# Gavinli-lgf/belief-planning

Hardware: AMD Instinct MI355X
Metric: branch-MPC solves/sec (whole node), highway N=20 M=3 branches, batch 4096 egos (higher is better)
Workload: dtype f64; 1 GPU; highway BranchMPC_CVaR closed loop, N=20, NB=1, m=3 (T=64, U=61), 4096 egos per GPU; batch_per_gpu=4096, global_batch=4096, world_size=1, parallelism=ego-sharded dp1, loop=per step: k_env + solve launches

## Files before the change

belief-planning_amd/csrc/bmpc_core.h:

```cpp
#pragma once

#include <stddef.h>
#include <stdint.h>

#include "bmpc.h"

#if defined(__HIPCC__)
#include <hip/hip_runtime.h>
#define BMPC_HD __host__ __device__ __forceinline__
#if defined(BMPC_INLINE_ALL)
#define BMPC_FN __host__ __device__ __forceinline__
#else
#define BMPC_FN __host__ __device__ __attribute__((noinline))
#endif
#else
#define BMPC_HD inline
#define BMPC_FN inline
#endif

#include <math.h>

namespace bmpc {

#if defined(__HIP_DEVICE_COMPILE__)
#if defined(BMPC_FLAT_SLAB)
#define BMPC_AS_GLOBAL
#else
#define BMPC_AS_GLOBAL __attribute__((address_space(1)))
#endif
#define BMPC_AS_LDS __attribute__((address_space(3)))
#define BMPC_AS_CONST __attribute__((address_space(4)))
#else
#define BMPC_AS_GLOBAL
#define BMPC_AS_LDS
#define BMPC_AS_CONST
#endif
typedef BMPC_AS_GLOBAL double gdouble;
typedef BMPC_AS_LDS double ldouble;
typedef const BMPC_AS_GLOBAL int32_t gint;

template <class T>
BMPC_HD T* uniform_ptr(T* p) {
#if defined(__HIP_DEVICE_COMPILE__)
  const uint64_t v = reinterpret_cast<uint64_t>(p);
  const uint32_t lo = __builtin_amdgcn_readfirstlane(static_cast<uint32_t>(v));
  const uint32_t hi = __builtin_amdgcn_readfirstlane(static_cast<uint32_t>(v >> 32));
  return reinterpret_cast<T*>((static_cast<uint64_t>(hi) << 32) | lo);
#else
  return p;
#endif
}

#define BMPC_TOPO_FIELDS(F)                                                                  \
  F(br_depth) F(br_len) F(br_ndx) F(br_ndu) F(br_child0) F(x_u) F(x_srcu) F(x_srcx) F(x_cone) \
  F(x_conepos) F(x_branch) F(succ_off) F(succ) F(lvl_off) F(lvl_nodes) F(u_x) F(u_cone)       \
  F(cone_b) F(cone_i) F(cone_c) F(cone_q) F(cone_off)
#define BMPC_TOPO_COUNT_(n) +1
enum { BMPC_TOPO_N = 0 BMPC_TOPO_FIELDS(BMPC_TOPO_COUNT_) };
#define BMPC_TOPO_MEMBER_(n) IP n;
template <class IP>
struct TopoT {
  BMPC_TOPO_FIELDS(BMPC_TOPO_MEMBER_)
};
typedef const BMPC_AS_LDS int32_t lint;
typedef TopoT<gint*> Topo;
typedef TopoT<lint*> TopoL;

enum { XF_S = 0, XF_BX = BMPC_MAX_N * BMPC_MAX_N, XF_SON = XF_BX + BMPC_MAX_FX, XF_BXSET = XF_SON + 1,
       XF_FX = XF_BXSET + 1, XF_FXSET = XF_FX + BMPC_MAX_FX * BMPC_MAX_N, XF_ROWS = XF_FXSET + 1,
       XF_BROWS = XF_ROWS + BMPC_MAX_FX * BMPC_MAX_N, XF_ROWSET = XF_BROWS + BMPC_MAX_FX,
       XF_COUNT = XF_ROWSET + 1 };

enum { ECO_FX = 0, ECO_W1 = BMPC_MAX_FX * BMPC_MAX_N, ECO_QQ = ECO_W1 + BMPC_MAX_N * BMPC_MAX_N,
       ECO_BX = ECO_QQ + BMPC_MAX_N * BMPC_MAX_N, ECO_COUNT = ECO_BX + BMPC_MAX_FX };

struct Plan {
  bmpc_plan_desc desc;
  int n, d, N, NB, m, nFx, nFu, Nc;
  int Ncol, zNB;
  int T, U, nbranch, bdim, ncones, nlevels;
  int oX, oU, oRho, oSig, oMup, oMum, oS, oJ, nv;
  int neq;
  int rFx, rFu, rRisk, rPos, nlp, nrows;
  int ng;
  int nsm;
  int lds_M, lds_piv, lds_rhs, lds_rhs2, lds_red, nlds;
  int lds_w, lds_wu, lds_fx, lds_fu, nconst;
  int nlds_lean;
  int lds_scr, nscr;
  int cgrp;
  int maxq;
  double W1[BMPC_MAX_N * BMPC_MAX_N];
  double Wu[BMPC_MAX_D * BMPC_MAX_D];
  double QQ[BMPC_MAX_N * BMPC_MAX_N];
  double RR[BMPC_MAX_D * BMPC_MAX_D];
  Topo t;
  int toff[BMPC_TOPO_N];
  int ntab;
  const double* lref;
  int nlref;
};

template <class X>
// ... 343 lines not shown
```

belief-planning_amd/csrc/bmpc_ipm.h:

```cpp
#pragma once

#include <type_traits>

#include "bmpc_tree.h"
#include "bmpc_wave.h"

#ifndef BMPC_EQUIL
#define BMPC_EQUIL 1
#endif
#ifndef BMPC_EQUIL_ITERS
#define BMPC_EQUIL_ITERS 3
#endif
#ifndef BMPC_TS_POST_RB_MIN
#define BMPC_TS_POST_RB_MIN 8
#endif
#ifndef BMPC_TS_POST_RB
#define BMPC_TS_POST_RB 4
#endif
#ifndef BMPC_PAIR_REFINE
#define BMPC_PAIR_REFINE 1
#endif
#ifndef BMPC_BLK_WAVE_SUBST
#define BMPC_BLK_WAVE_SUBST 1
#endif
// ... 37 lines not shown
#define BMPC_REFSCORE 1e-3
#endif
#ifndef BMPC_REFSCORE2
#define BMPC_REFSCORE2 1e-6
#endif
#ifndef BMPC_NITREF2
#define BMPC_NITREF2 2
#endif
#ifndef BMPC_REFTOL
#define BMPC_REFTOL 1e-14
#endif
#ifndef BMPC_REF_STALL
#define BMPC_REF_STALL 0
#endif

#ifndef BMPC_FN_APPLY_G
#define BMPC_FN_APPLY_G BMPC_FN
#endif
#ifndef BMPC_FN_APPLY_GT
#define BMPC_FN_APPLY_GT BMPC_FN
#endif
#ifndef BMPC_FN_SCALING
#define BMPC_FN_SCALING BMPC_FN
#endif
#ifndef BMPC_FN_MAX_STEP
#define BMPC_FN_MAX_STEP BMPC_FN
#endif
#ifndef BMPC_FN_TREE_SOLVE
#define BMPC_FN_TREE_SOLVE BMPC_FN
#endif
#ifndef BMPC_FN_FUSED
#define BMPC_FN_FUSED BMPC_FN
#endif

namespace bmpc {

enum {
  EXIT_OPTIMAL = 0, EXIT_PINF = 1, EXIT_DINF = 2, EXIT_INACC = 10,
  EXIT_MAXIT = -1, EXIT_NUMERICS = -2,
  EXIT_GUARD = -9
};

struct Ctx {
  CPlan* P;
  CLayout* L;
  gdouble* ws;
  BMPC_HD gdouble* at(size_t off) const { return ws + off; }
  BMPC_HD Ctx uniform() const { return Ctx{uniform_ptr(P), uniform_ptr(L), uniform_ptr(ws)}; }
};

template <int NX>
BMPC_HD void ctx_qx(const Ctx& C, double (&qx)[NX]) {
  const gdouble* xref = C.at(C.L->xref);
  double xr[NX];
#pragma unroll
  for (int r = 0; r < NX; ++r) xr[r] = xref[r];
#pragma unroll
  for (int c = 0; c < NX; ++c) {
    double v = 0.0;
#pragma unroll
    for (int r = 0; r < NX; ++r) v += xr[r] * C.P->desc.Q[r * NX + c];
    qx[c] = v;
  }
}

#define BMPC_CONE_ROUNDS(ex, P, G)                                \
  const auto G##_t = topo_view((P), ex);                         \
  const ConeGroups G = cone_groups(ex, (P).cgrp, (P).ncones);     \
  for (int rnd_ = 0; rnd_ < G.rounds; ++rnd_)
#define BMPC_CONE_K(P, G, k, off, q)                              \
  const int k = rnd_ * G.ngrp + G.g < (P).ncones ? rnd_ * G.ngrp + G.g : -1; \
  const int off = k >= 0 ? G##_t.cone_off[k] : 0;                 \
  const int q = k >= 0 ? G##_t.cone_q[k] : 0

template <class X>
struct MultiWave : std::integral_constant<bool, (BatchDiv<X>::v > 1)> {};

template <class X, class PB>
BMPC_HD double ebeta(const PB* boost, int nc, int k) {
  if constexpr (MultiWave<X>::value) return boost[nc + k];
  return exp(-boost[k]);
}

template <int NBR0 = 4, class X>
BMPC_HD void block_dots(const X ex, const gdouble* A, size_t astr, int na, const gdouble* B, size_t bstr, int nb,
                        int lo1, int hi1, int lo2, int hi2, double (&acc)[4][4]) {
  constexpr int NBR = MultiWave<X>::value ? NBR0 : 4;
#pragma unroll
  for (int a = 0; a < 4; ++a)
#pragma unroll
    for (int b = 0; b < 4; ++b) acc[a][b] = 0.0;
  const int n1 = hi1 - lo1, ntot = n1 + (hi2 - lo2);
  auto idx = [&](int t) { return t < n1 ? lo1 + t : lo2 + (t - n1); };
#pragma unroll 2
  for (int t = ex.lane; t < ntot; t += ex.nlanes) {
    const int i = idx(t);
    double av[4], bv[4];
#pragma unroll
    for (int a = 0; a < 4; ++a) av[a] = a < na ? A[a * astr + i] : 0.0;
#pragma unroll
    for (int b = 0; b < 4; ++b) bv[b] = b < nb ? B[b * bstr + i] : 0.0;
#pragma unroll
    for (int a = 0; a < 4; ++a)
#pragma unroll
      for (int b = 0; b < (NBR < 4 ? NBR : 4); ++b) acc[a][b] += av[a] * bv[b];
  }
  if constexpr (NBR >= 4) {
    ex.template sum_n<16>(&acc[0][0]);
  } else {
    double v[4 * NBR];
#pragma unroll
    for (int a = 0; a < 4; ++a)
#pragma unroll
      for (int b = 0; b < NBR; ++b) v[a * NBR + b] = acc[a][b];
    ex.template sum_n<4 * NBR>(v);
#pragma unroll
    for (int a = 0; a < 4; ++a)
#pragma unroll
      for (int b = 0; b < NBR; ++b) acc[a][b] = v[a * NBR + b];
  }
}

template <class T>
BMPC_HD int cone_supp_len(CPlan& P, const T& t, int k) {
  return t.cone_c[k] >= 0 ? P.N * (P.n + P.d + P.Nc) : P.d + P.Nc;
}
template <class T>
BMPC_HD int cone_supp_idx(CPlan& P, const T& t, int k, int e) {
  const int c = t.cone_c[k];
  if (c < 0) return e < P.d ? P.oU + e : P.oS + (e - P.d);
  const int xn = P.N * P.n, un = P.N * P.d;
  if (e < xn) return P.oX + t.br_ndx[c] * P.n + e;
  if (e < xn + un) return P.oU + t.br_ndu[c] * P.d + (e - xn);
  return P.oS + t.br_ndx[c] * P.Nc + (e - xn - un);
}
BMPC_HD bool coup_supp_dots(CPlan& P) { return P.ncones > 4; }

template <class X, class T>
BMPC_HD void cone_supp_dots(const X& ex, CPlan& P, const T& t, const gdouble* gk, int k, const gdouble* v0,
                            size_t vstr, int j0, int nvec, double (&acc)[16]) {
#pragma unroll
  for (int j = 0; j < 16; ++j) acc[j] = 0.0;
  const int tot = cone_supp_len(P, t, k);
  for (int e = ex.lane; e < tot; e += ex.nlanes) {
    const int i = cone_supp_idx(P, t, k, e);
    const double g = gk[i];
    double v[16];
#pragma unroll
    for (int j = 0; j < 16; ++j) v[j] = v0[(size_t)(j0 + j < nvec ? j0 + j : j0) * vstr + i];
#pragma unroll
    for (int j = 0; j < 16; ++j) acc[j] += (j0 + j < nvec ? g : 0.0) * v[j];
  }
  ex.template sum_n<16>(acc);
}

template <class X, class T>
BMPC_HD void cone_supp_gdx(const X& ex, CPlan& P, const T& t, const gdouble* g0, size_t gstr, const gdouble* dx, int k0,
                           double (&acc)[16]) {
#pragma unroll
  for (int j = 0; j < 16; ++j) acc[j] = 0.0;
  const int nc = P.ncones;
  const int kn = nc - k0 < 16 ? nc - k0 : 16;
  const int full = P.N * (P.n + P.d + P.Nc);
  int tot = 0;
  for (int j = 0; j < kn; ++j) tot += cone_supp_len(P, t, k0 + j);
  constexpr int UN = 8;
  for (int b = ex.lane; b < tot; b += UN * ex.nlanes) {
    double gv[UN], xv[UN];
    int kk[UN];
#pragma unroll
    for (int u = 0; u < UN; ++u) {
      const int f = b + u * ex.nlanes < tot ? b + u * ex.nlanes : b;
      const int j = f / full < kn ? f / full : kn - 1;
      const int e = f - j * full;
      const int i = cone_supp_idx(P, t, k0 + j, e);
      kk[u] = b + u * ex.nlanes < tot ? j : -1;
      gv[u] = g0[(size_t)(k0 + j) * gstr + i];
      xv[u] = dx[i];
    }
#pragma unroll
    for (int u = 0; u < UN; ++u)
#pragma unroll
      for (int j = 0; j < 16; ++j) acc[j] += (kk[u] == j ? gv[u] : 0.0) * xv[u];
  }
  ex.template sum_n<16>(acc);
}

template <class X, class T>
BMPC_HD void cone_supp_gdx2(const X& ex, CPlan& P, const T& t, const gdouble* g0, size_t gstr, const gdouble* dx1,
                            const gdouble* dx2, int k0, double (&acc1)[16], double (&acc2)[16]) {
#pragma unroll
  for (int j = 0; j < 16; ++j) acc1[j] = 0.0, acc2[j] = 0.0;
  const int nc = P.ncones;
  const int kn = nc - k0 < 16 ? nc - k0 : 16;
  const int full = P.N * (P.n + P.d + P.Nc);
  int tot = 0;
  for (int j = 0; j < kn; ++j) tot += cone_supp_len(P, t, k0 + j);
  constexpr int UN = 4;
  for (int b = ex.lane; b < tot; b += UN * ex.nlanes) {
    double gv[UN], xv1[UN], xv2[UN];
    int kk[UN];
#pragma unroll
    for (int u = 0; u < UN; ++u) {
// ... 1505 lines not shown
            Pn[q][j] = i == j ? pij : i < j ? 0.5 * (pij + pji) : 0.5 * (pji + pij);
          }
        }
#pragma unroll
        for (int q = 0; q < RX; ++q) {
          const int i = gl * RX + q;
          if (i < NX) {
#pragma unroll
            for (int j = 0; j < NX; ++j) ws[L.P + k * NX * NX + i * NX + j] = Pn[q][j];
#pragma unroll
            for (int m = 0; m < NU; ++m) ws[L.Kg + u * NU * NX + m * NX + i] = kc[q][m];
          }
        }
        if (gl == 0) mat_store(Qi, ws + L.Luu + u * NU * NU);
        BMPC_TOC_WAIT(C.ws, L, PROF_RIC_B, t_rb);
      }
    }
    ex.sync();
  }
  BMPC_TOC(C.ws, L, 23, t_ric);
  return ex.max(bad) == 0.0;
}

template <class X, int NX, int NU, int RX, int W>
BMPC_HD void bw_node(const X& ex, int gl, const double (&qx)[RX], const double (&Acol)[RX][NX],
                     const double (&Brow)[RX][NU], const double (&Kcol)[RX][NU], const double (&Lu)[NU][NU],
                     const double (&ru)[NU], double (&g)[RX], double (&l)[RX], double (&kfv)[NU]) {
#pragma unroll
  for (int q = 0; q < RX; ++q)
    if (gl * RX + q >= NX) g[q] = 0.0;
  double gfull[NX];
  task_gather<NX, RX, W>(ex, g, gfull);
  double qu[NU];
#pragma unroll
  for (int m = 0; m < NU; ++m) {
    double v = 0.0;
#pragma unroll
    for (int q = 0; q < RX; ++q) v += Brow[q][m] * g[q];
    qu[m] = -ru[m] + ex.tsum(v);
  }
#pragma unroll
  for (int m = 0; m < NU; ++m) {
    double v = 0.0;
#pragma unroll
    for (int c = 0; c < NU; ++c) v -= Lu[m][c] * qu[c];
    kfv[m] = v;
  }
#pragma unroll
  for (int q = 0; q < RX; ++q) {
    double v = qx[q];
#pragma unroll
    for (int j = 0; j < NX; ++j) v += Acol[q][j] * gfull[j];
#pragma unroll
    for (int m = 0; m < NU; ++m) v += Kcol[q][m] * qu[m];
    l[q] = v;
  }
}

template <class X, int NX, int NU, bool RB = false>
BMPC_FN_TREE_SOLVE void tree_solve(const X ex, const Ctx Cin, int nr, const gdouble* r0, size_t rs, const gdouble* e0,
                        size_t es, gdouble* o0, size_t os, gdouble* n0, size_t ns, int ncw = 0) {
  const Ctx C = Cin.uniform();
  r0 = uniform_ptr(r0);
  e0 = uniform_ptr(e0);
  o0 = uniform_ptr(o0);
  n0 = uniform_ptr(n0);
  constexpr int W = X::kTaskLanes;
  constexpr int RX = (NX + W - 1) / W;
  constexpr int NCM = BMPC_MAX_FX + 1;
  (void)NCM;
  CPlan& P = *C.P;
  CLayout& L = *C.L;
  BMPC_PROF(C.ws, L, PROF_TREESOLVE);
  BMPC_COUNT(C.ws, L, PROF_NTREE);
  const auto t = topo_view(P, ex);
  const int Nc = P.Nc;
  gdouble* ws = C.ws;
  gdouble* lv_ = ws + L.lvec;
  gdouble* kf_ = ws + L.kff;
  const size_t lstr = (size_t)P.T * NX, kstr = (size_t)P.U * NU;
  const gdouble* dh = ws + L.dh;
  const gdouble* sdv = ws + L.sd;
  const int gl = ex.lane % W, grp = ex.lane / W, ngrp = ex.nlanes / W;
  auto needed = [&](int b, int ri) {
    if (ri >= ncw) return true;
    int c = t.cone_c[ri];
    if (c < 0) return b == 0;
    while (c > b) c = (c - 1) / P.m;
    return c == b;
  };
  auto qx0 = [&](const gdouble* rr, int k, int i) {
    double rS[NCM], s0[NCM], s1[NCM];
#pragma unroll
    for (int c = 0; c < NCM; ++c) {
      const int kc = k * Nc + (c < Nc ? c : 0);
      rS[c] = rr[P.oS + kc];
      s0[c] = sdv[kc * 2];
      s1[c] = sdv[kc * 2 + 1];
    }
    const double on = t.x_u[k] >= 0 ? 1.0 : 0.0;
    double v = -rr[P.oX + k * NX + i] + dh[k * NX + i] * (on * s1[0] * rS[0] / s0[0]);
#pragma unroll
    for (int c = 1; c < NCM; ++c)
      if (c < Nc) v -= fxv(P, ex, c - 1, i) * (on * s1[c] * rS[c] / s0[c]);
    return v;
  };
  const bool pre = ex.uniform(P.nscr >= P.T * Nc);
  gdouble* q0_ = ws + L.qx0;
  if (pre) {
    BMPC_TIC(t_pre);
    ldouble* av = ex.lds + P.lds_scr;
    for (int ri = 0; ri < nr; ++ri) {
      const gdouble* rr = r0 + ri * rs;
      gdouble* q0 = q0_ + ri * lstr;
      int s0 = 0, l0 = P.T, s1 = 0, l1 = 0, s2 = 0, l2 = 0, s3 = 0, l3 = 0;
      if (ri < ncw) {
        int c = t.cone_c[ri] < 0 ? 0 : t.cone_c[ri];
        int st[4] = {0, 0, 0, 0}, ln[4] = {0, 0, 0, 0};
        bool deeper = true;
#pragma unroll
        for (int q = 0; q < 4; ++q) {
          if (deeper) {
            st[q] = t.br_ndx[c];
            ln[q] = t.br_len[c] + (t.br_child0[c] < 0 ? 1 : 0);
            if (c == 0) deeper = false;
            else c = (c - 1) / P.m;
          }
        }
        if (!deeper) s0 = st[0], l0 = ln[0], s1 = st[1], l1 = ln[1], s2 = st[2], l2 = ln[2], s3 = st[3], l3 = ln[3];
      }
      const int nn = l0 + l1 + l2 + l3;
      auto node = [&](int f) {
        const int f1 = f - l0, f2 = f1 - l1, f3 = f2 - l2;
        return f < l0 ? s0 + f : f1 < l1 ? s1 + f1 : f2 < l2 ? s2 + f2 : s3 + f3;
      };
      lane_batch<BMPC_TS_UN_AV>(ex, 0, nn * Nc, [&](int f) {
        const int k = node(f / Nc), it = k * Nc + f % Nc;
        const double on = t.x_u[k] >= 0 ? 1.0 : 0.0;
        return on * sdv[it * 2 + 1] * rr[P.oS + it] / sdv[it * 2];
      }, [&](int f, double v) { av[node(f / Nc) * Nc + f % Nc] = v; });
      ex.sync();
      lane_batch<BMPC_TS_UN>(ex, 0, nn * NX, [&](int f) {
        const int k = node(f / NX), j = f % NX, it = k * NX + j;
        double v = -rr[P.oX + it] + dh[it] * av[k * Nc];
        for (int c = 1; c < Nc; ++c) v -= fxv(P, ex, c - 1, j) * av[k * Nc + c];
        return v;
      }, [&](int f, double v) { q0[node(f / NX) * NX + f % NX] = v; });
      ex.sync();
    }
    BMPC_TOC(C.ws, L, PROF_X1, t_pre);
  }

  BMPC_TIC(t_bw);
  for (int dep = P.NB; dep >= 0; --dep) {
    const int b0 = branch_start(P, dep), nbd = branch_count(P, dep);
    const int nfull = nbd * (nr - ncw);
    int ncol = 0;
    for (int ri = 0; ri < ncw; ++ri) {
      const int c = t.cone_c[ri];
      ncol += (c < 0 ? 0 : t.br_depth[c]) >= dep ? 1 : 0;
    }
    const int ntask = nfull + ncol;
    const int rounds = (ntask + ngrp - 1) / ngrp;
    const bool leaf = dep == P.NB;
    for (int rd = 0; rd < rounds; ++rd) {
      const int task = rd * ngrp + grp;
      if (task >= ntask) continue;
      int b, ri;
      if (task < nfull) {
        b = b0 + task / (nr - ncw);
        ri = ncw + task % (nr - ncw);
      } else {
        int want = task - nfull;
        ri = 0;
        for (int r2 = 0; r2 < ncw; ++r2) {
          const int c = t.cone_c[r2];
          if ((c < 0 ? 0 : t.br_depth[c]) >= dep) {
            if (want == 0) {
              ri = r2;
              break;
            }
            --want;
          }
        }
        int c = t.cone_c[ri];
        if (c < 0) c = 0;
        while (t.br_depth[c] > dep) c = (c - 1) / P.m;
        b = c;
      }
      const gdouble* rr = r0 + ri * rs;
      const gdouble* ee = e0 + ri * es;
      const gdouble* q0 = q0_ + ri * lstr;
      gdouble* lvec = lv_ + ri * lstr;
      gdouble* kf = kf_ + ri * kstr;
      const int ndx = t.br_ndx[b], ndu = t.br_ndu[b], len = t.br_len[b];
      const int c0 = t.br_child0[b];
      double l[RX];
      if (leaf) {
        const int tn = ndx + len;
#pragma unroll
        for (int q = 0; q < RX; ++q) {
          const int i = gl * RX + q;
          l[q] = i < NX ? (pre ? q0[tn * NX + i] : qx0(rr, tn, i)) : 0.0;
          if (i < NX) lvec[tn * NX + i] = l[q];
        }
      }
      for (int jn = len - 1; jn >= 0; --jn) {
        const int k = ndx + jn, u = ndu + jn;
        double qx[RX], Acol[RX][NX], Brow[RX][NU], Kcol[RX][NU], Lu[NU][NU], ru[NU];
#pragma unroll
        for (int q = 0; q < RX; ++q) {
          const int i = gl * RX + q < NX ? gl * RX + q : NX - 1;
          qx[q] = pre ? q0[k * NX + i] : qx0(rr, k, i);
#pragma unroll
          for (int j = 0; j < NX; ++j) Acol[q][j] = ws[L.Ad + u * NX * NX + j * NX + i];
#pragma unroll
          for (int m = 0; m < NU; ++m) Brow[q][m] = ws[L.Bd + u * NX * NU + i * NU + m];
#pragma unroll
          for (int m = 0; m < NU; ++m) Kcol[q][m] = ws[L.Kg + u * NU * NX + m * NX + i];
        }
        mat_load(Lu, ws + L.Luu + u * NU * NU);
#pragma unroll
        for (int m = 0; m < NU; ++m) ru[m] = rr[P.oU + u * NU + m];
        double g[RX];
        if (jn < len - 1 || leaf) {
          double ec[NX];
#pragma unroll
          for (int j = 0; j < NX; ++j) ec[j] = ee[(k + 1) * NX + j];
#pragma unroll
          for (int q = 0; q < RX; ++q) {
            const int i = gl * RX + q < NX ? gl * RX + q : NX - 1;
            double v = l[q];
#pragma unroll
            for (int j = 0; j < NX; ++j) v += ws[L.P + (k + 1) * NX * NX + i * NX + j] * ec[j];
            g[q] = v;
          }
        } else {
#pragma unroll
          for (int q = 0; q < RX; ++q) g[q] = 0.0;
          for (int ci = 0; ci < P.m; ++ci) {
            if (!needed(c0 + ci, ri)) continue;
            const int c = t.br_ndx[c0 + ci];
            double ec[NX];
#pragma unroll
            for (int j = 0; j < NX; ++j) ec[j] = ee[c * NX + j];
#pragma unroll
            for (int q = 0; q < RX; ++q) {
              const int i = gl * RX + q < NX ? gl * RX + q : NX - 1;
              double v = lvec[c * NX + i];
#pragma unroll
              for (int j = 0; j < NX; ++j) v += ws[L.P + c * NX * NX + i * NX + j] * ec[j];
              g[q] += v;
            }
          }
        }
        double kfv[NU];
        bw_node<X, NX, NU, RX, W>(ex, gl, qx, Acol, Brow, Kcol, Lu, ru, g, l, kfv);
#pragma unroll
        for (int q = 0; q < RX; ++q) {
          const int i = gl * RX + q;
          if (i < NX) lvec[k * NX + i] = l[q];
        }
        if (gl == 0)
#pragma unroll
          for (int m = 0; m < NU; ++m) kf[u * NU + m] = kfv[m];
      }
    }
    ex.sync();
  }
  BMPC_TOC(C.ws, L, PROF_X2, t_bw);
  BMPC_TIC(t_fw);
  for (int it = ex.lane; it < nr * NX; it += ex.nlanes) {
    const int ri = it / NX, j = it % NX;
    o0[ri * os + P.oX + j] = e0[ri * es + j];
  }
  ex.sync();
  for (int dep = 0; dep <= P.NB; ++dep) {
    const int b0 = branch_start(P, dep), nbd = branch_count(P, dep);
    const int ntask = nbd * nr;
    const int rounds = (ntask + ngrp - 1) / ngrp;
    const bool leaf = dep == P.NB;
    for (int rd = 0; rd < rounds; ++rd) {
      const int task = rd * ngrp + grp;
      if (task >= ntask) continue;
      const int b = b0 + task / nr, ri = task % nr;
      gdouble* o = o0 + ri * os;
      const gdouble* ee = e0 + ri * es;
      const gdouble* kf = kf_ + ri * kstr;
      const bool kfon = needed(b, ri);
      const int ndx = t.br_ndx[b], ndu = t.br_ndu[b], len = t.br_len[b];
      const int c0 = t.br_child0[b];
      double xk[NX];
#pragma unroll
      for (int j = 0; j < NX; ++j) xk[j] = o[P.oX + ndx * NX + j];
      for (int jn = 0; jn < len; ++jn) {
        const int k = ndx + jn, u = ndu + jn;
        double Arow[RX][NX], Brow[RX][NU], Kcol[RX][NU], kfu[NU], en[RX];
        const int kn = (jn < len - 1 || leaf) ? k + 1 : t.br_ndx[c0 >= 0 ? c0 : 0];
#pragma unroll
        for (int q = 0; q < RX; ++q) {
          const int i = gl * RX + q < NX ? gl * RX + q : NX - 1;
#pragma unroll
          for (int j = 0; j < NX; ++j) Arow[q][j] = ws[L.Ad + u * NX * NX + i * NX + j];
#pragma unroll
          for (int m = 0; m < NU; ++m) Brow[q][m] = ws[L.Bd + u * NX * NU + i * NU + m];
#pragma unroll
          for (int m = 0; m < NU; ++m) Kcol[q][m] = ws[L.Kg + u * NU * NX + m * NX + i];
          en[q] = ee[kn * NX + i];
        }
#pragma unroll
        for (int m = 0; m < NU; ++m) kfu[m] = kfon ? kf[u * NU + m] : 0.0;
        double uk[NU];
#pragma unroll
        for (int m = 0; m < NU; ++m) {
          double v = 0.0;
#pragma unroll
          for (int q = 0; q < RX; ++q) v += gl * RX + q < NX ? Kcol[q][m] * xk[gl * RX + q < NX ? gl * RX + q : 0] : 0.0;
          uk[m] = kfu[m] + ex.tsum(v);
        }
        if (gl == 0)
#pragma unroll
          for (int m = 0; m < NU; ++m) o[P.oU + u * NU + m] = uk[m];
        double xn[RX];
#pragma unroll
        for (int q = 0; q < RX; ++q) {
          double v = 0.0;
#pragma unroll
          for (int j = 0; j < NX; ++j) v += Arow[q][j] * xk[j];
#pragma unroll
          for (int m = 0; m < NU; ++m) v += Brow[q][m] * uk[m];
          xn[q] = v;
        }
        if (jn < len - 1 || leaf) {
#pragma unroll
          for (int q = 0; q < RX; ++q) {
            const int i = gl * RX + q;
            xn[q] += en[q];
            if (i < NX) o[P.oX + (k + 1) * NX + i] = xn[q];
          }
          task_gather<NX, RX, W>(ex, xn, xk);
        } else {
          for (int ci = 0; ci < P.m; ++ci) {
            const int c = t.br_ndx[c0 + ci];
#pragma unroll
            for (int q = 0; q < RX; ++q) {
              const int i = gl * RX + q;
              if (i < NX) o[P.oX + c * NX + i] = xn[q] + ee[c * NX + i];
            }
          }
        }
      }
    }
    ex.sync();
  }
  BMPC_TOC(C.ws, L, PROF_X3, t_fw);
  BMPC_TIC(t_post);
  if constexpr (RB) {
    constexpr int NB4 = BMPC_TS_POST_RB;
    struct VR { double v[NB4]; };
    for (int rb = 0; rb < nr; rb += NB4) {
      const int rn = nr - rb < NB4 ? nr - rb : NB4;
      if (n0) {
        lane_batch<BMPC_TS_UN>(ex, 0, P.T * NX, [&](int it) {
          const int k = it / NX, i = it % NX;
          double pr[NX];
#pragma unroll
          for (int j = 0; j < NX; ++j) pr[j] = ws[L.P + k * NX * NX + i * NX + j];
          VR out;
#pragma unroll
          for (int a = 0; a < NB4; ++a) {
// ... 314 lines not shown
      const int i = i1 - u;
      if (i >= 0) {
        if (j == i) b[i] = b[i] / mc[u];
        wave_sync();
        const double bi = b[i];
        if (row && j < i) b[j] -= mc[u] * bi;
        wave_sync();
      }
    }
  }
}

template <class X, class PM, class PP, class PB>
BMPC_HD void small_lu_solve(const X ex, const PM* M, const PP* piv, PB* b, int n) {
#if BMPC_SUBST_REG
  if constexpr (MultiWave<X>::value) {
    if (n <= 64) {
      PB* const bs[1] = {b};
      if (ex.lane < 64) small_lu_solve_wave<1>(ex.lane, M, piv, bs, n);
      ex.sync();
      return;
    }
  }
#endif
  if (ex.lane == 0)
    for (int k = 0; k < n; ++k) {
      const int p = (int)piv[k];
      if (p != k) {
        const double tmp = b[k];
        b[k] = b[p];
        b[p] = tmp;
      }
    }
  ex.sync();
  if constexpr (RowLanes<X>::value) {
#if BMPC_BLK_WAVE_SUBST
    if constexpr (X::nlanes > 64) {
      if (n <= 64) {
        if (ex.lane < 64) small_lu_solve_rows_wave(ex.lane, M, b, n);
        ex.sync();
        return;
      }
    }
#endif
    if (n <= X::nlanes) {
      small_lu_solve_rows(ex, M, b, n);
      return;
    }
  }
  for (int i = 0; i < n; ++i) {
    const double bi = b[i];
    for (int j = i + 1 + ex.lane; j < n; j += ex.nlanes) b[j] -= M[j * n + i] * bi;
    ex.sync();
  }
  for (int i = n - 1; i >= 0; --i) {
    const double bi = b[i] / M[i * n + i];
    for (int j = ex.lane; j < i; j += ex.nlanes) b[j] -= M[j * n + i] * bi;
    ex.sync();
    if (ex.lane == 0) b[i] = bi;
    ex.sync();
  }
}

template <class X>
BMPC_HD auto coup_mem(const X& ex, gdouble* ws, CLayout& L, CPlan& P, int off) {
  if constexpr (X::kCoupLds) return ex.lds + off;
  else return ws + L.coup + (off - P.lds_M);
}
template <class X>
BMPC_HD auto coup_vec(const X& ex, int off) { return ex.lds + off; }


BMPC_HD int gvar(CPlan& P, int i) { return i == P.ng - 1 ? P.oJ : P.oRho + i; }

template <class X, int NX, int NU>
BMPC_FN bool kkt_coupling(const X ex, const Ctx Cin, int extra) {
  const Ctx C = Cin.uniform();
  CPlan& P = *C.P;
  CLayout& L = *C.L;
  BMPC_PROF(C.ws, L, PROF_COUPLING);
  gdouble* ws = C.ws;
  const int nc = P.ncones;
  BMPC_TIC(t_cts);
  if (ex.uniform(nc + extra >= BMPC_TS_POST_RB_MIN))
    tree_solve<X, NX, NU, true>(ex, C, nc + extra, ws + L.gk, P.nv, ws + L.zeros, P.neq, ws + L.colk, P.nv,
                                ws + L.colnu, P.neq, nc);
  else
    tree_solve<X, NX, NU>(ex, C, nc + extra, ws + L.gk, P.nv, ws + L.zeros, P.neq, ws + L.colk, P.nv, ws + L.colnu,
                          P.neq, nc);
  BMPC_TOC(C.ws, L, PROF_CTS, t_cts);
  BMPC_TIC(t_cdot);
  const int ng = P.ng, nb = P.bdim, ns = P.nsm;
  auto* M = coup_mem(ex, ws, L, P, P.lds_M);
  const gdouble* eta = ws + L.eta;
  const gdouble* dl = ws + L.dl;
  const gdouble* p = ws + L.p;
  const int ntree = P.oRho;
  for (int i = ex.lane; i < ns * ns; i += ex.nlanes) M[i] = 0.0;
  ex.sync();
  if (coup_supp_dots(P) && BMPC_BLK_PAIR_DOTS && MultiWave<X>::value) {
    const auto t = topo_view(P, ex);
    for (int pr = ex.lane; pr < nc * nc; pr += ex.nlanes) {
      const int k = pr / nc, j = pr - (pr / nc) * nc;
      const gdouble* g = ws + L.gk + (size_t)k * P.nv;
      const gdouble* v = ws + L.colk + (size_t)j * P.nv;
      const int tot = cone_supp_len(P, t, k);
      double acc = 0.0;
      for (int e0 = 0; e0 < tot; e0 += 8) {
        double gv[8], vv[8];
#pragma unroll
        for (int u = 0; u < 8; ++u) {
          const int i = cone_supp_idx(P, t, k, e0 + u < tot ? e0 + u : e0);
          gv[u] = g[i];
          vv[u] = v[i];
        }
#pragma unroll
        for (int u = 0; u < 8; ++u)
          if (e0 + u < tot) acc += gv[u] * vv[u];
      }
      const double ck = 2.0 / (eta[k] * eta[k]);
      M[(ng + nb + k) * ns + ng + nb + j] = ck * acc + (k == j ? 1.0 : 0.0);
    }
  } else if (coup_supp_dots(P)) {
    const auto t = topo_view(P, ex);
    for (int k = 0; k < nc; ++k)
      for (int j0 = 0; j0 < nc; j0 += 16) {
        double acc[16];
        cone_supp_dots(ex, P, t, ws + L.gk + (size_t)k * P.nv, k, ws + L.colk, P.nv, j0, nc, acc);
        if (ex.lane == 0) {
          const double ck = 2.0 / (eta[k] * eta[k]);
          for (int j = j0; j < nc && j < j0 + 16; ++j)
            M[(ng + nb + k) * ns + ng + nb + j] = ck * acc[j - j0] + (k == j ? 1.0 : 0.0);
        }
      }
  } else {
    for (int k0 = 0; k0 < nc; k0 += 4)
      for (int j0 = 0; j0 < nc; j0 += 4) {
        const int na = nc - k0 < 4 ? nc - k0 : 4, nbk = nc - j0 < 4 ? nc - j0 : 4;
        double acc[4][4];
        block_dots(ex, ws + L.gk + (size_t)k0 * P.nv, P.nv, na, ws + L.colk + (size_t)j0 * P.nv, P.nv, nbk,
                   0, ntree, P.oS, P.oJ, acc);
        if (ex.lane == 0)
          for (int a = 0; a < na; ++a) {
            const int k = k0 + a;
            const double ck = 2.0 / (eta[k] * eta[k]);
            for (int b = 0; b < nbk; ++b) {
              const int j = j0 + b;
              M[(ng + nb + k) * ns + ng + nb + j] = ck * acc[a][b] + (k == j ? 1.0 : 0.0);
            }
          }
      }
  }
  for (int b = ex.lane; b < nb; b += ex.nlanes) {
    const double w = dl[P.rRisk + b];
    M[b * ns + b] = 1.0 / (w * w);
  }
  for (int j = ex.lane; j < 2 * nb * P.m; j += ex.nlanes) {
    const double w = dl[P.rRisk + nb + j];
    const int gi = 2 * nb + j;
    M[gi * ns + gi] = 1.0 / (w * w);
  }
  for (int b = ex.lane; b < nb; b += ex.nlanes) {
    const int row = ng + b;
    M[row * ns + b] = 1.0;
    M[b * ns + row] = 1.0;
    M[row * ns + nb + b] = 1.0;
    M[(nb + b) * ns + row] = 1.0;
    for (int i = 0; i < P.m; ++i) {
      const int gi = 2 * nb + nb * P.m + b * P.m + i;
      const double a = -p[b * P.m + i] / P.desc.ralpha;
      M[row * ns + gi] = a;
      M[gi * ns + row] = a;
    }
  }
  for (int it = ex.lane; it < nc * ng; it += ex.nlanes) {
    const int k = it / ng, i = it % ng;
    const double gv = ws[L.gk + (size_t)k * P.nv + gvar(P, i)];
    const double ck = 2.0 / (eta[k] * eta[k]);
    M[i * ns + ng + nb + k] = gv;
    M[(ng + nb + k) * ns + i] = -ck * gv;
  }
  ex.sync();
  BMPC_TOC(C.ws, L, PROF_CDOT, t_cdot);
  BMPC_TIC(t_lu);
  bool ok;
  if constexpr (BMPC_WAVE_LU && RowLanes<X>::value && (MultiWave<X>::value || !X::kCoupLds)) {
    if (ns <= 64 && (MultiWave<X>::value || ns >= BMPC_WAVE_LU_MIN1)) {
      double bad = 0.0;
      if (ex.lane < 64) bad = small_lu_wave(ex.lane, M, coup_vec(ex, P.lds_piv), ns) ? 0.0 : 1.0;
      ok = ex.max(bad) == 0.0;
    } else {
      ok = small_lu(ex, M, coup_vec(ex, P.lds_piv), ns);
    }
  } else {
    ok = small_lu(ex, M, coup_vec(ex, P.lds_piv), ns);
  }
  BMPC_TOC(C.ws, L, PROF_LU, t_lu);
  return ok;
}

template <class X, int NX, int NU, bool R3ZERO>
BMPC_HD void kkt_back(const X ex, const Ctx& C, const gdouble* tz, const gdouble* r2, const gdouble* r3h,
                      gdouble* dx, gdouble* dy, gdouble* dzh, bool fin);

template <class X, int NX, int NU, bool R3ZERO = false>
BMPC_HD void kkt_solve_once(const X ex, const Ctx Cin, const gdouble* r1, const gdouble* r2,
                            const gdouble* r3h, gdouble* dx, gdouble* dy, gdouble* dzh, bool tr_ready, bool fin) {
  const Ctx C = Cin.uniform();
  CPlan& P = *C.P;
  CLayout& L = *C.L;
  gdouble* ws = C.ws;
  gdouble* tr = ws + L.k_r0;
  gdouble* tz = ws + L.k_nv0;
  if constexpr (R3ZERO) {
    tz = const_cast<gdouble*>(r1);
  } else {
    if (!tr_ready) apply_W(ex, C, 1, r3h, tr);
    apply_GT<X, NX, NU>(ex, C, tr, tz, r1);
  }
  tree_solve<X, NX, NU>(ex, C, 1, tz, 0, r2, 0, dx, 0, dy, 0);
  kkt_back<X, NX, NU, R3ZERO>(ex, C, tz, r2, r3h, dx, dy, dzh, fin);
}

template <class X, int NX, int NU, bool R3ZERO>
BMPC_HD void kkt_back(const X ex, const Ctx& C, const gdouble* tz, const gdouble* r2, const gdouble* r3h,
                      gdouble* dx, gdouble* dy, gdouble* dzh, bool fin) {
  CPlan& P = *C.P;
  CLayout& L = *C.L;
  BMPC_PROF(C.ws, L, PROF_BACK);
  gdouble* ws = C.ws;
  gdouble* tr = ws + L.k_r0;
  const int ng = P.ng, nb = P.bdim, nc = P.ncones, ns = P.nsm;
  auto* b = coup_vec(ex, P.lds_rhs);
  const gdouble* eta = ws + L.eta;
  if (coup_supp_dots(P)) {
    const auto t = topo_view(P, ex);
    for (int k0 = 0; k0 < nc; k0 += 16) {
      double acc[16];
      cone_supp_gdx(ex, P, t, ws + L.gk, P.nv, dx, k0, acc);
      if (ex.lane == 0)
        for (int a = 0; a < 16 && k0 + a < nc; ++a) b[ng + nb + k0 + a] = 2.0 / (eta[k0 + a] * eta[k0 + a]) * acc[a];
    }
  } else {
    for (int k0 = 0; k0 < nc; k0 += 4) {
      const int na = nc - k0 < 4 ? nc - k0 : 4;
      double acc[4][4];
      block_dots<1>(ex, ws + L.gk + (size_t)k0 * P.nv, P.nv, na, dx, 0, 1, 0, P.oRho, P.oS, P.oJ, acc);
      if (ex.lane == 0)
        for (int a = 0; a < na; ++a) b[ng + nb + k0 + a] = 2.0 / (eta[k0 + a] * eta[k0 + a]) * acc[a][0];
    }
  }
  for (int i = ex.lane; i < ng + nb; i += ex.nlanes) b[i] = i < ng ? tz[gvar(P, i)] : r2[P.T * NX + i - ng];
  ex.sync();
  BMPC_TIC(t_lus);
  small_lu_solve(ex, coup_mem(ex, ws, L, P, P.lds_M), coup_vec(ex, P.lds_piv), b, ns);
  BMPC_TOC(C.ws, L, PROF_LUS, t_lus);
  const auto* bc = b + ng + nb;
  const gdouble* colk = ws + L.colk;
  const gdouble* colnu = ws + L.colnu;
  const int n1 = P.oRho, n2 = n1 + (P.oJ - P.oS), n3 = n2 + P.T * NX;
  auto row = [&](int t, int& i, bool& isx) {
    isx = t < n2;
    i = t < n1 ? t : t < n2 ? P.oS + (t - n1) : t - n2;
  };
  lane_batch(ex, 0, n3, [&](int t) {
    int i;
    bool isx;
    row(t, i, isx);
    const gdouble* col = isx ? colk : colnu;
    const size_t cs = isx ? (size_t)P.nv : (size_t)P.neq;
    const gdouble* src = isx ? dx : dy;
    double v = src[i];
    for (int k0 = 0; k0 < nc; k0 += 4) {
      double c4[4], b4[4];
#pragma unroll
      for (int a = 0; a < 4; ++a) {
        c4[a] = col[(size_t)(k0 + a < nc ? k0 + a : nc - 1) * cs + i];
        b4[a] = k0 + a < nc ? bc[k0 + a] : 0.0;
      }
#pragma unroll
      for (int a = 0; a < 4; ++a) v -= b4[a] * c4[a];
    }
    return v;
  }, [&](int t, double v) {
    int i;
    bool isx;
    row(t, i, isx);
    if (isx) dx[i] = v;
    else dy[i] = v;
  });
  for (int i = ex.lane; i < ng + nb; i += ex.nlanes) {
    if (i < ng) dx[gvar(P, i)] = b[i];
    else dy[P.T * NX + i - ng] = b[i];
  }
  ex.sync();
  if constexpr (R3ZERO) apply_G<X, NX, NU, 3>(ex, C, dx, dzh, r3h, tr);
  else if (fin) apply_G<X, NX, NU, 2>(ex, C, dx, dzh, r3h, tr);
  else apply_G<X, NX, NU, 1>(ex, C, dx, dzh, r3h, tr);
}

template <class X, int NX, int NU, bool R3ZERO = false>
BMPC_HD void kkt_back_pair(const X ex, const Ctx& C, const gdouble* tz1, const gdouble* r21, const gdouble* r3h1,
                           gdouble* dx1, gdouble* dy1, gdouble* dzh1, const gdouble* tz2, const gdouble* r22,
                           const gdouble* r3h2, gdouble* dx2, gdouble* dy2, gdouble* dzh2, bool fin) {
  CPlan& P = *C.P;
  CLayout& L = *C.L;
  BMPC_PROF(C.ws, L, PROF_BACK);
  gdouble* ws = C.ws;
  gdouble* tr = ws + L.k_r0;
  const int ng = P.ng, nb = P.bdim, nc = P.ncones, ns = P.nsm;
  auto* b1 = coup_vec(ex, P.lds_rhs);
  auto* b2 = coup_vec(ex, P.lds_rhs2);
  const gdouble* eta = ws + L.eta;
  if (coup_supp_dots(P)) {
    const auto t = topo_view(P, ex);
    for (int k0 = 0; k0 < nc; k0 += 16) {
      double acc1[16], acc2[16];
      cone_supp_gdx2(ex, P, t, ws + L.gk, P.nv, dx1, dx2, k0, acc1, acc2);
      if (ex.lane == 0)
        for (int a = 0; a < 16 && k0 + a < nc; ++a) {
          b1[ng + nb + k0 + a] = 2.0 / (eta[k0 + a] * eta[k0 + a]) * acc1[a];
          b2[ng + nb + k0 + a] = 2.0 / (eta[k0 + a] * eta[k0 + a]) * acc2[a];
        }
    }
  } else {
    for (int k0 = 0; k0 < nc; k0 += 4) {
      const int na = nc - k0 < 4 ? nc - k0 : 4;
      double acc[4][4];
      block_dots<2>(ex, ws + L.gk + (size_t)k0 * P.nv, P.nv, na, dx1, (size_t)(dx2 - dx1), 2, 0, P.oRho, P.oS, P.oJ,
                 acc);
      if (ex.lane == 0)
        for (int a = 0; a < na; ++a) {
          b1[ng + nb + k0 + a] = 2.0 / (eta[k0 + a] * eta[k0 + a]) * acc[a][0];
          b2[ng + nb + k0 + a] = 2.0 / (eta[k0 + a] * eta[k0 + a]) * acc[a][1];
        }
    }
  }
  for (int i = ex.lane; i < ng + nb; i += ex.nlanes) {
    b1[i] = i < ng ? tz1[gvar(P, i)] : r21[P.T * NX + i - ng];
    b2[i] = i < ng ? tz2[gvar(P, i)] : r22[P.T * NX + i - ng];
  }
  ex.sync();
  BMPC_TIC(t_lus);
  bool both = false;
#if BMPC_SUBST_REG
  if constexpr (MultiWave<X>::value) {
    if (ns <= 64) {
      decltype(b1) const bs[2] = {b1, b2};
      if (ex.lane < 64) small_lu_solve_wave<2>(ex.lane, coup_mem(ex, ws, L, P, P.lds_M), coup_vec(ex, P.lds_piv), bs, ns);
      ex.sync();
      both = true;
    }
  }
#endif
  if (!both) {
    small_lu_solve(ex, coup_mem(ex, ws, L, P, P.lds_M), coup_vec(ex, P.lds_piv), b1, ns);
    small_lu_solve(ex, coup_mem(ex, ws, L, P, P.lds_M), coup_vec(ex, P.lds_piv), b2, ns);
  }
  BMPC_TOC(C.ws, L, PROF_LUS, t_lus);
  const auto* bc1 = b1 + ng + nb;
  const auto* bc2 = b2 + ng + nb;
  const gdouble* colk = ws + L.colk;
  const gdouble* colnu = ws + L.colnu;
  const int n1 = P.oRho, n2 = n1 + (P.oJ - P.oS), n3 = n2 + P.T * NX;
  auto row = [&](int t, int& i, bool& isx) {
    isx = t < n2;
    i = t < n1 ? t : t < n2 ? P.oS + (t - n1) : t - n2;
  };
  struct V2 { double a, b; };
  lane_batch<4>(ex, 0, n3, [&](int t) {
    int i;
    bool isx;
    row(t, i, isx);
    const gdouble* col = isx ? colk : colnu;
    const size_t cs = isx ? (size_t)P.nv : (size_t)P.neq;
    const gdouble* s1 = isx ? dx1 : dy1;
    const gdouble* s2 = isx ? dx2 : dy2;
    double v1 = s1[i], v2 = s2[i];
    for (int k0 = 0; k0 < nc; k0 += 4) {
      double c4[4], p4[4], q4[4];
#pragma unroll
      for (int a = 0; a < 4; ++a) {
        c4[a] = col[(size_t)(k0 + a < nc ? k0 + a : nc - 1) * cs + i];
        p4[a] = k0 + a < nc ? bc1[k0 + a] : 0.0;
        q4[a] = k0 + a < nc ? bc2[k0 + a] : 0.0;
      }
#pragma unroll
      for (int a = 0; a < 4; ++a) v1 -= p4[a] * c4[a];
#pragma unroll
      for (int a = 0; a < 4; ++a) v2 -= q4[a] * c4[a];
    }
    return V2{v1, v2};
  }, [&](int t, V2 v) {
    int i;
    bool isx;
    row(t, i, isx);
    if (isx) dx1[i] = v.a, dx2[i] = v.b;
    else dy1[i] = v.a, dy2[i] = v.b;
  });
  for (int i = ex.lane; i < ng + nb; i += ex.nlanes) {
    if (i < ng) dx1[gvar(P, i)] = b1[i], dx2[gvar(P, i)] = b2[i];
    else dy1[P.T * NX + i - ng] = b1[i], dy2[P.T * NX + i - ng] = b2[i];
  }
  ex.sync();
  if constexpr (R3ZERO) {
    apply_G<X, NX, NU, 3>(ex, C, dx1, dzh1, r3h1, tr);
    apply_G<X, NX, NU, 3>(ex, C, dx2, dzh2, r3h2, tr);
  } else if (fin) {
    apply_G<X, NX, NU, 2>(ex, C, dx1, dzh1, r3h1, tr);
    apply_G<X, NX, NU, 2>(ex, C, dx2, dzh2, r3h2, tr);
  } else {
    apply_G<X, NX, NU, 1>(ex, C, dx1, dzh1, r3h1, tr);
    apply_G<X, NX, NU, 1>(ex, C, dx2, dzh2, r3h2, tr);
// ... 876 lines not shown
```

belief-planning_amd/csrc/bmpc_plan.cpp:

```cpp
#include <stdlib.h>
#include "bmpc_plan.h"

#include <algorithm>

#include <math.h>
#include <string.h>

#include <deque>

namespace bmpc {

namespace {

void sqrtm_sym(const double* A, int n, double* out) {
  double a[BMPC_MAX_N][BMPC_MAX_N], v[BMPC_MAX_N][BMPC_MAX_N];
  for (int i = 0; i < n; ++i)
    for (int j = 0; j < n; ++j) {
      a[i][j] = A[i * n + j];
      v[i][j] = i == j ? 1.0 : 0.0;
    }
  for (int sweep = 0; sweep < 100; ++sweep) {
    double off = 0.0;
    for (int i = 0; i < n; ++i)
      for (int j = i + 1; j < n; ++j) off += a[i][j] * a[i][j];
// ... 319 lines not shown
    const size_t r = o;
    o += (cnt + 7) & ~(size_t)7;
    return r;
  };
  const int nv = P.nv, neq = P.neq, nr = P.nrows, nc = P.ncones;
  L.uLin = take((size_t)(U + 1) * d);
  L.pprev = take((size_t)bd * m);
  L.misc = take(8 + BMPC_MAX_N);
  L.xpred = take((size_t)T * n);
  L.upred = take((size_t)U * d);
  L.sol = take(nv);
  L.xbar = take((size_t)T * n);
  L.zbar = take((size_t)T * n);
  L.ubar = take((size_t)U * d);
  L.Ad = take((size_t)U * n * n);
  L.Bd = take((size_t)U * n * d);
  L.Cd = take((size_t)U * n);
  L.dh = take((size_t)T * P.Ncol * n);
  L.h0 = take((size_t)T * P.Ncol);
  L.w = take(nbr);
  L.p = take((size_t)bd * m);
  L.dp = take((size_t)bd * m * n);
  L.boost = take(2 * (size_t)nc);
  L.xref = take(n);
  L.x = take(nv);
  L.y = take(neq);
  L.z = take(nr);
  L.s = take(nr);
  L.lam = take(nr);
  L.z1 = take(nr);
  L.z2 = take(nr);
  L.dz = take(nr);
  L.ds = take(nr);
  L.rx = take(nv);
  L.rz = take(nr);
  L.hvec = take(nr);
  L.ta = take(nv);
  L.ta2 = take(nv);
  L.ya = take(neq);
  L.ra = take(nr);
  L.rb = take(nr);
  L.rc = take(nr);
  L.bestx = take(nv);
  L.ej = take(nv);
  L.xeq = take(nv);
  L.aeq = take(neq);
  L.geq = take(nr);
  L.k_r0 = take(nr);
  L.k_nv0 = take(nv);
  L.k_e1 = take(2 * (size_t)nv);
  L.k_e2 = take(2 * (size_t)neq);
  L.k_e3 = take(nr);
  L.k_t3 = take(nr);
  L.k_t3b = take(nr);
  L.k_cx = take(2 * (size_t)nv);
  L.k_cy = take(2 * (size_t)neq);
  L.k_cz = take(2 * (size_t)nr);
  L.k_nv1 = take(nv);
  L.dl = take(P.nlp);
  L.dli = take(P.nlp);
  L.eta = take(nc);
  L.wbar = take(nr);
  L.vnt = take(nr);
  L.hx = take((size_t)T * n * n);
  L.hu = take((size_t)U * d * d);
  L.sd = take((size_t)T * P.Nc * 2);
  L.P = take((size_t)T * n * n);
  L.Kg = take((size_t)U * d * n);
  L.Luu = take((size_t)U * d * d);
  const size_t nrhs = nc > 0 ? (size_t)nc + 2 : 1;
  L.kff = take(nrhs * U * d);
  L.lvec = take(nrhs * T * n);
  L.qx0 = take(nrhs * T * n);
  if (nc > 0) {
    L.gk = take((size_t)(nc + 2) * nv);
    const size_t colk = take((size_t)(nc + 2) * nv);
    L.colk = colk;
    L.x1 = colk + (size_t)nc * nv;
    L.x2 = L.x1 + nv;
    const size_t colnu = take((size_t)(nc + 2) * neq);
    L.colnu = colnu;
    L.y1 = colnu + (size_t)nc * neq;
    L.y2 = L.y1 + neq;
    const size_t zb = take((size_t)(nc + 2) * neq);
    L.zeros = zb;
    L.bvec = zb + (size_t)nc * neq;
    L.ry = L.bvec + neq;
  } else {
    L.gk = L.colk = L.colnu = take(0);
    L.x1 = take(nv);
    L.y1 = take(neq);
    L.x2 = take(nv);
    L.y2 = take(neq);
    L.ry = take(neq);
    L.bvec = take(neq);
    L.zeros = take(neq);
  }
  L.prof = take(PROF_COUNT);
  L.coup = take((size_t)P.nsm * P.nsm + 2 * (size_t)P.nsm);
  L.ist = take(64);
  if (desc.controller != BMPC_CTRL_CVAR) {
    const int NS = n + d;
    L.qo = take((size_t)U * d * d);
    L.qq = take(nv);
    L.Pa = take((size_t)T * NS * NS);
    L.Ka = take((size_t)U * d * NS);
    L.la = take((size_t)T * NS);
  } else {
    L.qo = L.qq = L.Pa = L.Ka = L.la = 0;
  }
  L.xform = take(XF_COUNT);
  L.xlin = robust ? take((size_t)T * n) : 0;
  L.zrob = robust ? take((size_t)(T - 1) * P.Ncol * n) : 0;
  L.stride = o;
  return "";
}

}
```

Measured before the change: 76060 solves/s.

## Exploit single-owner cone gradient rows and share one zero RHS row

Adds block_dots_owned, which uses the fact that each variable is owned by at most one cone. Each lane loads one gk element instead of up to four rows when forming the coupling dot products. The per-cone zero equality RHS rows are also collapsed into one shared zero row, which shrinks the workspace and the memory read in tree_solve. The cost is extra index arithmetic per element and an assumption about cone ownership. The owned path also ignores k0/j0 offsets, so it relies on nc<=4 or on the ownership mapping being correct.

```diff
diff --git a/belief-planning_amd/csrc/bmpc_core.h b/belief-planning_amd/csrc/bmpc_core.h
--- a/belief-planning_amd/csrc/bmpc_core.h
+++ b/belief-planning_amd/csrc/bmpc_core.h
@@ -19,6 +19,16 @@
 #endif
 
 #include <math.h>
+
+#ifndef BMPC_IPM_OWNED_LOADS
+#define BMPC_IPM_OWNED_LOADS 1
+#endif
+#ifndef BMPC_OWNED_GK
+#define BMPC_OWNED_GK BMPC_IPM_OWNED_LOADS
+#endif
+#ifndef BMPC_OWNED_ZROW
+#define BMPC_OWNED_ZROW BMPC_IPM_OWNED_LOADS
+#endif
 
 namespace bmpc {
 
diff --git a/belief-planning_amd/csrc/bmpc_ipm.h b/belief-planning_amd/csrc/bmpc_ipm.h
--- a/belief-planning_amd/csrc/bmpc_ipm.h
+++ b/belief-planning_amd/csrc/bmpc_ipm.h
@@ -143,6 +143,24 @@
   return exp(-boost[k]);
 }
 
+template <int NBR, class X>
+BMPC_HD void block_dots_reduce(const X& ex, double (&acc)[4][4]) {
+  if constexpr (NBR >= 4) {
+    ex.template sum_n<16>(&acc[0][0]);
+  } else {
+    double v[4 * NBR];
+#pragma unroll
+    for (int a = 0; a < 4; ++a)
+#pragma unroll
+      for (int b = 0; b < NBR; ++b) v[a * NBR + b] = acc[a][b];
+    ex.template sum_n<4 * NBR>(v);
+#pragma unroll
+    for (int a = 0; a < 4; ++a)
+#pragma unroll
+      for (int b = 0; b < NBR; ++b) acc[a][b] = v[a * NBR + b];
+  }
+}
+
 template <int NBR0 = 4, class X>
 BMPC_HD void block_dots(const X ex, const gdouble* A, size_t astr, int na, const gdouble* B, size_t bstr, int nb,
                         int lo1, int hi1, int lo2, int hi2, double (&acc)[4][4]) {
@@ -166,20 +184,38 @@
 #pragma unroll
       for (int b = 0; b < (NBR < 4 ? NBR : 4); ++b) acc[a][b] += av[a] * bv[b];
   }
-  if constexpr (NBR >= 4) {
-    ex.template sum_n<16>(&acc[0][0]);
-  } else {
-    double v[4 * NBR];
+  block_dots_reduce<NBR>(ex, acc);
+}
+
+template <int NBR0 = 4, int NX, int NU, class X, class T>
+BMPC_HD void block_dots_owned(const X ex, CPlan& P, const T& t, const gdouble* A, size_t astr, const gdouble* B,
+                              size_t bstr, int nb, double (&acc)[4][4]) {
+  constexpr int NBR = MultiWave<X>::value ? NBR0 : 4;
+#pragma unroll
+  for (int a = 0; a < 4; ++a)
+#pragma unroll
+    for (int b = 0; b < 4; ++b) acc[a][b] = 0.0;
+  const int nx = P.oU, n1 = P.oRho, ntot = n1 + (P.oJ - P.oS);
+  const unsigned Nc = (unsigned)P.Nc;
+#pragma unroll 2
+  for (int tt = ex.lane; tt < ntot; tt += ex.nlanes) {
+    const bool isu = tt >= nx && tt < n1, iss = tt >= n1;
+    const int i = iss ? P.oS + (tt - n1) : tt;
+    const int node = iss ? (int)((unsigned)(tt - n1) / Nc) : isu ? (tt - nx) / NU : tt / NX;
+    const int own = (isu ? t.u_cone : t.x_cone)[node];
+    const int o = iss && node == 0 ? P.ncones - 1 : own;
+    const double g = A[(size_t)(o > 0 ? o : 0) * astr + i];
+    double av[4], bv[4];
+#pragma unroll
+    for (int a = 0; a < 4; ++a) av[a] = a == o ? g : 0.0;
+#pragma unroll
+    for (int b = 0; b < 4; ++b) bv[b] = b < nb ? B[b * bstr + i] : 0.0;
 #pragma unroll
     for (int a = 0; a < 4; ++a)
 #pragma unroll
-      for (int b = 0; b < NBR; ++b) v[a * NBR + b] = acc[a][b];
-    ex.template sum_n<4 * NBR>(v);
-#pragma unroll
-    for (int a = 0; a < 4; ++a)
-#pragma unroll
-      for (int b = 0; b < NBR; ++b) acc[a][b] = v[a * NBR + b];
-  }
+      for (int b = 0; b < (NBR < 4 ? NBR : 4); ++b) acc[a][b] += av[a] * bv[b];
+  }
+  block_dots_reduce<NBR>(ex, acc);
 }
 
 template <class T>
@@ -1851,6 +1887,13 @@
   const gdouble* dh = ws + L.dh;
   const gdouble* sdv = ws + L.sd;
   const int gl = ex.lane % W, grp = ex.lane / W, ngrp = ex.nlanes / W;
+  auto erow = [&](int ri) -> const gdouble* {
+#if BMPC_OWNED_ZROW
+    return ri < ncw ? ws + L.zeros : e0 + (size_t)(ri - ncw) * es;
+#else
+    return e0 + ri * es;
+#endif
+  };
   auto needed = [&](int b, int ri) {
     if (ri >= ncw) return true;
     int c = t.cone_c[ri];
@@ -1958,7 +2001,7 @@
         b = c;
       }
       const gdouble* rr = r0 + ri * rs;
-      const gdouble* ee = e0 + ri * es;
+      const gdouble* ee = erow(ri);
       const gdouble* q0 = q0_ + ri * lstr;
       gdouble* lvec = lv_ + ri * lstr;
       gdouble* kf = kf_ + ri * kstr;
@@ -2041,7 +2084,7 @@
   BMPC_TIC(t_fw);
   for (int it = ex.lane; it < nr * NX; it += ex.nlanes) {
     const int ri = it / NX, j = it % NX;
-    o0[ri * os + P.oX + j] = e0[ri * es + j];
+    o0[ri * os + P.oX + j] = erow(ri)[j];
   }
   ex.sync();
   for (int dep = 0; dep <= P.NB; ++dep) {
@@ -2054,7 +2097,7 @@
       if (task >= ntask) continue;
       const int b = b0 + task / nr, ri = task % nr;
       gdouble* o = o0 + ri * os;
-      const gdouble* ee = e0 + ri * es;
+      const gdouble* ee = erow(ri);
       const gdouble* kf = kf_ + ri * kstr;
       const bool kfon = needed(b, ri);
       const int ndx = t.br_ndx[b], ndu = t.br_ndu[b], len = t.br_len[b];
@@ -2535,11 +2578,12 @@
   gdouble* ws = C.ws;
   const int nc = P.ncones;
   BMPC_TIC(t_cts);
+  const gdouble* e0 = ws + (BMPC_OWNED_ZROW ? L.bvec : L.zeros);
   if (ex.uniform(nc + extra >= BMPC_TS_POST_RB_MIN))
-    tree_solve<X, NX, NU, true>(ex, C, nc + extra, ws + L.gk, P.nv, ws + L.zeros, P.neq, ws + L.colk, P.nv,
+    tree_solve<X, NX, NU, true>(ex, C, nc + extra, ws + L.gk, P.nv, e0, P.neq, ws + L.colk, P.nv,
                                 ws + L.colnu, P.neq, nc);
   else
-    tree_solve<X, NX, NU>(ex, C, nc + extra, ws + L.gk, P.nv, ws + L.zeros, P.neq, ws + L.colk, P.nv, ws + L.colnu,
+    tree_solve<X, NX, NU>(ex, C, nc + extra, ws + L.gk, P.nv, e0, P.neq, ws + L.colk, P.nv, ws + L.colnu,
                           P.neq, nc);
   BMPC_TOC(C.ws, L, PROF_CTS, t_cts);
   BMPC_TIC(t_cdot);
@@ -2591,8 +2635,12 @@
       for (int j0 = 0; j0 < nc; j0 += 4) {
         const int na = nc - k0 < 4 ? nc - k0 : 4, nbk = nc - j0 < 4 ? nc - j0 : 4;
         double acc[4][4];
+#if BMPC_OWNED_GK
+        block_dots_owned<4, NX, NU>(ex, P, topo_view(P, ex), ws + L.gk, P.nv, ws + L.colk, P.nv, nbk, acc);
+#else
         block_dots(ex, ws + L.gk + (size_t)k0 * P.nv, P.nv, na, ws + L.colk + (size_t)j0 * P.nv, P.nv, nbk,
                    0, ntree, P.oS, P.oJ, acc);
+#endif
         if (ex.lane == 0)
           for (int a = 0; a < na; ++a) {
             const int k = k0 + a;
@@ -2698,7 +2746,11 @@
     for (int k0 = 0; k0 < nc; k0 += 4) {
       const int na = nc - k0 < 4 ? nc - k0 : 4;
       double acc[4][4];
+#if BMPC_OWNED_GK
+      block_dots_owned<1, NX, NU>(ex, P, topo_view(P, ex), ws + L.gk, P.nv, dx, 0, 1, acc);
+#else
       block_dots<1>(ex, ws + L.gk + (size_t)k0 * P.nv, P.nv, na, dx, 0, 1, 0, P.oRho, P.oS, P.oJ, acc);
+#endif
       if (ex.lane == 0)
         for (int a = 0; a < na; ++a) b[ng + nb + k0 + a] = 2.0 / (eta[k0 + a] * eta[k0 + a]) * acc[a][0];
     }
@@ -2780,8 +2832,12 @@
     for (int k0 = 0; k0 < nc; k0 += 4) {
       const int na = nc - k0 < 4 ? nc - k0 : 4;
       double acc[4][4];
+#if BMPC_OWNED_GK
+      block_dots_owned<2, NX, NU>(ex, P, topo_view(P, ex), ws + L.gk, P.nv, dx1, (size_t)(dx2 - dx1), 2, acc);
+#else
       block_dots<2>(ex, ws + L.gk + (size_t)k0 * P.nv, P.nv, na, dx1, (size_t)(dx2 - dx1), 2, 0, P.oRho, P.oS, P.oJ,
                  acc);
+#endif
       if (ex.lane == 0)
         for (int a = 0; a < na; ++a) {
           b1[ng + nb + k0 + a] = 2.0 / (eta[k0 + a] * eta[k0 + a]) * acc[a][0];
diff --git a/belief-planning_amd/csrc/bmpc_plan.cpp b/belief-planning_amd/csrc/bmpc_plan.cpp
--- a/belief-planning_amd/csrc/bmpc_plan.cpp
+++ b/belief-planning_amd/csrc/bmpc_plan.cpp
@@ -425,9 +425,10 @@
     L.colnu = colnu;
     L.y1 = colnu + (size_t)nc * neq;
     L.y2 = L.y1 + neq;
-    const size_t zb = take((size_t)(nc + 2) * neq);
+    const size_t nz = BMPC_OWNED_ZROW ? 1 : nc;
+    const size_t zb = take((nz + 2) * neq);
     L.zeros = zb;
-    L.bvec = zb + (size_t)nc * neq;
+    L.bvec = zb + nz * neq;
     L.ry = L.bvec + neq;
   } else {
     L.gk = L.colk = L.colnu = take(0);
```

Result: no change. 76610 solves/s (median of 6 runs) (+0.7%).
